# ps-auxw/CLI-P

Hardware: AMD Instinct MI355X
Metric: images/sec ViT-B/32 encode (higher is better)
Workload: dtype bf16

## Files before the change

cli-p_amd/_lib.py:

```python
import ctypes as C
import os

HERE = os.path.dirname(os.path.abspath(__file__))
DEV_LIB = os.environ.get("CLIPMI_DEV_LIB", "") not in ("", "0")
LIB_PATH = os.path.join(HERE, "libclipmi_dev.so" if DEV_LIB else "libclipmi.so")

ABI_VERSION = 8
F32, BF16, U8 = 0, 1, 2

SYMBOLS = [
    "clipmi_encode_image_workspace_bytes", "clipmi_encode_image",
    "clipmi_encode_text_workspace_bytes", "clipmi_encode_text",
    "clipmi_topk_ip_workspace_bytes", "clipmi_topk_ip",
    "clipmi_topk_ip_coarse_workspace_bytes", "clipmi_topk_ip_coarse", "clipmi_dbg_topk_coarse_scan_ms",
    "clipmi_rows_stats", "clipmi_rows_absmax", "clipmi_rows_order_workspace_bytes", "clipmi_rows_order_by_absmax", "clipmi_rows_to_bf16", "clipmi_i8_copy_bytes", "clipmi_i8_meta_bytes", "clipmi_quantize_rows_i8", "clipmi_topk_ip_coarse_i8", "clipmi_dbg_topk_coarse_i8_scan_ms",
    "clipmi_topk_ip_wide_workspace_bytes", "clipmi_topk_ip_wide_i8", "clipmi_dbg_topk_wide_i8_scan_ms",
    "clipmi_dbg_quantize_rows_fp8", "clipmi_dbg_gemm_fp8",
    "clipmi_merge_topk_workspace_bytes", "clipmi_merge_topk", "clipmi_merge_topk_packed",
    "clipmi_l2_normalize_rows", "clipmi_resize_crop_rgb8", "clipmi_jpeg_workspace_bytes", "clipmi_jpeg_decode_rgb8", "clipmi_jpeg_progressive_workspace_bytes", "clipmi_jpeg_decode_progressive_rgb8", "clipmi_png_workspace_bytes", "clipmi_png_decode_rgb8", "clipmi_last_error", "clipmi_abi_version",
    "clipmi_dbg_gemm_bf16", "clipmi_dbg_layernorm", "clipmi_dbg_attention", "clipmi_dbg_topk_scan_ms",
    "clipmi_dbg_encode_image_probe_ms", "clipmi_dbg_encode_image_probe3_ms",
    "clipmi_dbg_split_stats", "clipmi_dbg_gemm_ln", "clipmi_dbg_gemm_resid_ln", "clipmi_dbg_gemm_resid_ln_leaf", "clipmi_dbg_gemm_ln_leaf", "clipmi_dbg_quantize_rows_fp8mx", "clipmi_dbg_gemm_fp8_bsa",
]


class Tower(C.Structure):
    _fields_ = [(n, C.c_int32) for n in (
        "abi_version", "kind", "width", "layers", "heads", "mlp", "embed", "tokens",
        "patch", "res", "patch_k", "vocab")] + [(n, C.c_uint64) for n in (
        "blob_bytes",
        "off_patch_w", "off_cls", "off_pos", "off_ln_pre_w", "off_ln_pre_b",
        "off_tok_emb",
        "off_layers", "layer_stride",
        "lo_ln1_w", "lo_ln1_b", "lo_qkv_w", "lo_qkv_b", "lo_out_w", "lo_out_b",
        "lo_ln2_w", "lo_ln2_b", "lo_fc_w", "lo_fc_b", "lo_proj_w", "lo_proj_b",
        "off_ln_post_w", "off_ln_post_b", "off_out_proj")] + [
        ("weight_format", C.c_int32), ("ln_fold", C.c_int32)] + [(n, C.c_uint64) for n in (
        "lo_qkv_s", "lo_out_s", "lo_fc_s", "lo_proj_s", "lo_qkv_colsum", "lo_qkv_cb", "lo_fc_colsum", "lo_fc_cb")]


class ClipmiError(RuntimeError):
    pass

# ... 93 lines not shown
    L.clipmi_png_workspace_bytes.argtypes = [i32, i64]
    L.clipmi_png_decode_rgb8.restype = i32
    L.clipmi_png_decode_rgb8.argtypes = [vp, vp, i32, i64, i64, vp, vp, vp, i64, vp]
    L.clipmi_dbg_gemm_bf16.restype = i32
    L.clipmi_dbg_gemm_bf16.argtypes = [vp, vp, vp, vp, i32, i32, i32, i32, vp]
    L.clipmi_dbg_split_stats.restype = i32
    L.clipmi_dbg_split_stats.argtypes = [vp, i32, vp, vp, i32, i32, vp]
    L.clipmi_dbg_gemm_ln.restype = i32
    L.clipmi_dbg_gemm_ln.argtypes = [vp, vp, vp, vp, vp, vp, i32, i32, i32, i32, vp]
    L.clipmi_dbg_quantize_rows_fp8mx.restype = i32
    L.clipmi_dbg_quantize_rows_fp8mx.argtypes = [vp, vp, vp, i32, i32, vp]
    L.clipmi_dbg_gemm_fp8_bsa.restype = i32
    L.clipmi_dbg_gemm_fp8_bsa.argtypes = [vp, vp, vp, vp, vp, vp, i32, i32, i32, i32, vp]
    L.clipmi_dbg_gemm_resid_ln_leaf.restype = i32
    L.clipmi_dbg_gemm_resid_ln_leaf.argtypes = [vp, vp, vp, vp, vp, i32, i32, i32, vp]
    L.clipmi_dbg_gemm_ln_leaf.restype = i32
    L.clipmi_dbg_gemm_ln_leaf.argtypes = [vp, vp, vp, vp, vp, vp, i32, i32, i32, i32, vp]
    L.clipmi_dbg_gemm_resid_ln.restype = i32
    L.clipmi_dbg_gemm_resid_ln.argtypes = [vp, vp, vp, vp, vp, vp, i32, i32, i32, i32, vp]
    L.clipmi_dbg_layernorm.restype = i32
    L.clipmi_dbg_layernorm.argtypes = [vp, vp, vp, vp, i32, i32, i32, vp]
    L.clipmi_dbg_attention.restype = i32
    L.clipmi_dbg_attention.argtypes = [vp, vp, i32, i32, i32, i32, vp]
    L.clipmi_dbg_topk_scan_ms.restype = i32
    L.clipmi_dbg_topk_scan_ms.argtypes = [vp, i64, i32, vp, i32, i32, vp, vp, vp, sz, vp, i32, C.POINTER(C.c_float)]
    L.clipmi_dbg_encode_image_probe_ms.restype = i32
    L.clipmi_dbg_encode_image_probe_ms.argtypes = [TP, vp, vp, i32, i32, vp, vp, sz, vp, i32, i32,
                                                   C.POINTER(C.c_float), C.POINTER(C.c_int)]
    L.clipmi_dbg_encode_image_probe3_ms.restype = i32
    L.clipmi_dbg_encode_image_probe3_ms.argtypes = [TP, vp, vp, i32, i32, vp, vp, sz, vp, i32, i32,
                                                    C.POINTER(C.c_float), C.POINTER(C.c_int), C.POINTER(C.c_int),
                                                    C.POINTER(C.c_int)]
    if L.clipmi_abi_version() != ABI_VERSION:
        raise ClipmiError(f"libclipmi.so ABI {L.clipmi_abi_version()} != binding {ABI_VERSION}: rebuild")
    _lib = L
    return L


def check(rc, what):
    if rc != 0:
        msg = lib().clipmi_last_error().decode("utf-8", "replace")
        raise ClipmiError(f"{what} failed (code {rc}): {msg}")


def last_error():
    return lib().clipmi_last_error().decode("utf-8", "replace")
# ... 31 lines not shown
```

cli-p_amd/csrc/encode.hip:

```cpp
#include "vit_kernels.hpp"

namespace clipmi {
namespace {

struct Ws {
    unsigned short* patches;
    float* x;
    unsigned short* h;
    unsigned short* big;
    unsigned short* pooled;
    int* rowidx;
    unsigned char* a8;
    float* a_scale;
    unsigned char* a_bs;
    unsigned char* x8;
    unsigned char* x8_bs;
    void* x3;
    float* ln_part;
    float* ln_leaf;
    void* x3c;
    float* partc;
    float* leafc;
    float* xc;
};

size_t carve(const clipmi_tower* t, int B, void* base, size_t cap, Ws* out) {
    Arena ar(base ? base : reinterpret_cast<void*>(256), cap);
    const size_t rows = (size_t)B * t->tokens;
    const int W = t->width;
    Ws w{};
    if (t->kind == 0) w.patches = ar.take<unsigned short>((size_t)B * (t->tokens - 1) * t->patch_k);
    w.x = ar.take<float>(rows * W);
    w.h = ar.take<unsigned short>(rows * W);
    w.big = ar.take<unsigned short>(rows * 4 * W);
    w.pooled = ar.take<unsigned short>((size_t)B * W);
    w.rowidx = ar.take<int>((size_t)B);
    if (t->weight_format == 1) {
        w.a8 = ar.take<unsigned char>(rows * 4 * W);
        w.a_scale = ar.take<float>(rows);
        w.a_bs = ar.take<unsigned char>((rows + 255) / 256 * 256 * (size_t)(4 * W / 32));
    }
    if (t->ln_fold && t->weight_format == 1) {
        w.x8 = ar.take<unsigned char>(rows * W);
        w.x8_bs = ar.take<unsigned char>((rows + 255) / 256 * 256 * (size_t)(W / 32));
        w.ln_part = ar.take<float>(rows * 2 * (W / 256));
    } else if (t->ln_fold) {
        w.x3 = ar.take<unsigned char>(rows * resid_row_bytes(W));
        w.ln_part = ar.take<float>(rows * 2 * (W / 256));
        if (rows <= (size_t)SKINNY_MAX_M) w.ln_leaf = ar.take<float>(rows * 2 * (W / 4));
    }
    if (t->kind == 0 && t->weight_format == 0) {
        if (t->ln_fold) {
            w.x3c = ar.take<unsigned char>((size_t)B * resid_row_bytes(W));
            w.partc = ar.take<float>((size_t)B * 2 * (W / 256));
            if (B <= SKINNY_MAX_M) w.leafc = ar.take<float>((size_t)B * 2 * (W / 4));
        } else {
            w.xc = ar.take<float>((size_t)B * W);
        }
    }
    if (out) *out = w;
    return ar.off + 256;
}

int check_tower(const clipmi_tower* t, int kind, const char* who) {
    if (!t) return set_err(CLIPMI_EINVAL, "%s: NULL tower", who);
    if (t->abi_version != CLIPMI_ABI_VERSION)
        return set_err(CLIPMI_EINVAL, "%s: tower ABI %d != %d", who, t->abi_version, CLIPMI_ABI_VERSION);
    if (t->kind != kind) return set_err(CLIPMI_EINVAL, "%s: tower kind %d", who, t->kind);
    if (t->width % 128 != 0 || t->heads * 64 != t->width || t->mlp != 4 * t->width || t->embed % 128 != 0 ||
        t->width > 1024 || t->layers < 1)
        return set_err(CLIPMI_EUNSUPPORTED,
                       "%s: width=%d heads=%d mlp=%d embed=%d (need width %% 128 == 0 <= 1024, head dim 64, embed %% 128 == 0)",
                       who, t->width, t->heads, t->mlp, t->embed);
    if (t->weight_format != 0 && t->weight_format != 1)
        return set_err(CLIPMI_EINVAL, "%s: weight_format %d", who, t->weight_format);
    if (t->weight_format == 1 && t->width % 256 != 0)
        return set_err(CLIPMI_EUNSUPPORTED, "%s: fp8 weights need width %% 256 == 0 (width %d)", who, t->width);
    if (t->ln_fold != 0 && (t->ln_fold != 1 || t->width % 256 != 0))
        return set_err(CLIPMI_EINVAL, "%s: ln_fold %d needs width %% 256 == 0 (width %d)", who, t->ln_fold, t->width);
#ifndef CLIPMI_DEV
    if (t->ln_fold != 0 && t->weight_format != 0)
        return set_err(CLIPMI_EUNSUPPORTED, "%s: folded LayerNorms on FP8 weights exist in the development library only", who);
#endif
    if (t->tokens > 80 && kind == 1)
        return set_err(CLIPMI_EUNSUPPORTED, "%s: %d tokens (causal attention covers <= 80)", who, t->tokens);
    return 0;
}

template <typename T>
const T* at(const void* blob, uint64_t off) {
    return reinterpret_cast<const T*>(static_cast<const char*>(blob) + off);
}

bool encode_tail() {
    static const int mode = (int)dev_knob("CLIPMI_ENCODE_TAIL", 1);
    return mode != 0;
}

int launch_gather_rows(const void* src, void* dst, int B, int L, size_t row_bytes, hipStream_t st) {
    if (row_bytes % 16 != 0) return set_err(CLIPMI_EINVAL, "gather_rows: %zu bytes per row", row_bytes);
    const int row16 = (int)(row_bytes / 16);
    hipLaunchKernelGGL(gather_rows_kernel, dim3((unsigned)(((long long)B * row16 + 255) / 256)), dim3(256), 0, st,
                       static_cast<const uint4*>(src), static_cast<uint4*>(dst), B, L, row16);
    CLIPMI_CHECK_LAUNCH("gather_rows_kernel");
    return 0;
}

int run_layers(const clipmi_tower* t, const void* blob, const Ws& w, int B, int causal, hipStream_t st, GemmProbe* probe,
               bool* pruned = nullptr) {
    const int W = t->width, L = t->tokens, M = B * L;
    const bool fp8 = t->weight_format == 1;
    const bool tail = pruned && !causal && !fp8 && (t->ln_fold ? w.x3c != nullptr : w.xc != nullptr) && encode_tail();
    if (pruned) *pruned = tail;
    auto linear = [&](const unsigned short* A, int K, uint64_t w_off, uint64_t b_off, void* out, int N, int epi) -> int {
        GemmArgs g{};
        g.bias = at<float>(blob, b_off); g.out = out; g.M = M; g.N = N; g.K = K;
        g.A = A; g.W = at<unsigned short>(blob, w_off);
        return launch_gemm_algo(g, epi, 0, st, probe);
    };
#ifdef CLIPMI_DEV
    if (t->ln_fold && fp8) {
        auto lnfold8 = [&](uint64_t w_off, uint64_t s_off, uint64_t cb_off, uint64_t cs_off, void* out, unsigned char* out_bs, int N,
                           int epi) -> int {
            GemmArgs g{};
            g.A = reinterpret_cast<const unsigned short*>(w.x8); g.a_bscale = w.x8_bs;
            g.W = at<unsigned short>(blob, w_off); g.w_scale = at<float>(blob, s_off);
            g.bias = at<float>(blob, cb_off); g.colsum = at<float>(blob, cs_off); g.ln_part_in = w.ln_part;
// ... 32 lines not shown
    if (t->ln_fold) {
        auto lb_of = [&](int l) { return t->off_layers + (uint64_t)l * t->layer_stride; };
        const bool leaf_mode = w.ln_leaf != nullptr && gemm_resid_writes_leaves(M, W, W) && gemm_resid_writes_leaves(M, W, 4 * W);
        bool leaves = false;
        auto ln_linear = [&](uint64_t w_off, uint64_t cb_off, uint64_t cs_off, int N, int epi) -> int {
            GemmArgs g{};
            g.A = static_cast<const unsigned short*>(w.x3); g.lda_bytes = (unsigned)resid_row_bytes(W);
            g.W = at<unsigned short>(blob, w_off); g.bias = at<float>(blob, cb_off);
            g.colsum = at<float>(blob, cs_off); g.ln_part_in = w.ln_part;
            if (leaves) g.ln_leaf_in = w.ln_leaf;
            g.out = w.big; g.M = M; g.N = N; g.K = W;
            return launch_gemm_algo(g, epi, 0, st, probe);
        };
        auto resid_linear = [&](const unsigned short* A, int K, uint64_t w_off, uint64_t b_off) -> int {
            GemmArgs g{};
            g.A = A; g.W = at<unsigned short>(blob, w_off); g.bias = at<float>(blob, b_off);
            g.M = M; g.N = W; g.K = K;
            g.x3 = w.x3; g.ln_part = w.ln_part; g.tmp_f32 = w.x;
            if (leaf_mode) { g.ln_leaf = w.ln_leaf; leaves = true; }
            return launch_gemm_algo(g, EPI_BIAS_RESID_LN_F32, 0, st, probe);
        };
        for (int l = 0; l < t->layers; ++l) {
            const uint64_t lb = lb_of(l);
            if (int rc = ln_linear(lb + t->lo_qkv_w, lb + t->lo_qkv_cb, lb + t->lo_qkv_colsum, 3 * W, EPI_LN_BIAS_BF16)) return rc;
            if (tail && l == t->layers - 1) {
                const bool tleaf = w.leafc != nullptr && gemm_resid_writes_leaves(B, W, W) && gemm_resid_writes_leaves(B, W, 4 * W);
                if (int rc = launch_attention(w.big, w.h, B, L, t->heads, causal, 1, st)) return rc;
                if (int rc = launch_gather_rows(w.x3, w.x3c, B, L, resid_row_bytes(W), st)) return rc;
                auto tail_resid = [&](const unsigned short* A, unsigned lda_bytes, int K, uint64_t w_off, uint64_t b_off) -> int {
                    GemmArgs g{};
                    g.A = A; g.lda_bytes = lda_bytes; g.W = at<unsigned short>(blob, w_off); g.bias = at<float>(blob, b_off);
                    g.M = B; g.N = W; g.K = K;
                    g.x3 = w.x3c; g.ln_part = w.partc; g.tmp_f32 = w.x;
                    if (tleaf) g.ln_leaf = w.leafc;
                    return launch_gemm_algo(g, EPI_BIAS_RESID_LN_F32, 0, st, nullptr);
                };
                if (int rc = tail_resid(w.h, (unsigned)((size_t)L * W * 2), W, lb + t->lo_out_w, lb + t->lo_out_b)) return rc;
                GemmArgs g{};
                g.A = static_cast<const unsigned short*>(w.x3c); g.lda_bytes = (unsigned)resid_row_bytes(W);
                g.W = at<unsigned short>(blob, lb + t->lo_fc_w); g.bias = at<float>(blob, lb + t->lo_fc_cb);
                g.colsum = at<float>(blob, lb + t->lo_fc_colsum); g.ln_part_in = w.partc;
                if (tleaf) g.ln_leaf_in = w.leafc;
                g.out = w.big; g.M = B; g.N = 4 * W; g.K = W;
                if (int rc = launch_gemm_algo(g, EPI_LN_BIAS_QGELU_BF16, 0, st, nullptr)) return rc;
                return tail_resid(w.big, 0u, 4 * W, lb + t->lo_proj_w, lb + t->lo_proj_b);
            }
            hipEvent_t* aev = nullptr;
            if (probe && probe->mode == 2 && probe->n < GemmProbe::MAX) {
                const int pi = probe->begin(GemmProbe::EPI_ATTENTION, 2, st, 0);
                aev = &probe->ev[2 * pi];
            }
// ... 256 lines not shown
```

cli-p_amd/csrc/vit_kernels.hip:

```cpp
#include "vit_kernels.hpp"
#include <hip/hip_ext.h>
#include <cstdlib>

namespace clipmi {

int launch_layernorm(const LnArgs& a, hipStream_t st) {
    if (a.M < 1) return 0;
    if (a.W % 4 != 0 || a.W > 1024) return set_err(CLIPMI_EINVAL, "layernorm: W=%d (need W %% 4 == 0, W <= 1024)", a.W);
    if (a.out_x3 && (a.W % 256 != 0 || !a.out_part)) return set_err(CLIPMI_EINVAL, "layernorm: split output needs W %% 256 == 0");
    hipLaunchKernelGGL(layernorm_kernel, dim3((a.M + 3) / 4), dim3(256), 0, st, a);
    CLIPMI_CHECK_LAUNCH("layernorm_kernel");
    return 0;
}

int launch_split_stats(const float* x_or_add, bool add, void* x3, float* part, int M, int W, hipStream_t st) {
    if (M < 1) return 0;
    if (!x_or_add || !x3 || !part || W % 256 != 0 || W < 256 || W > 1024)
        return set_err(CLIPMI_EINVAL, "split_stats: W=%d (need W %% 256 == 0, 256 <= W <= 1024)", W);
    if (add) hipLaunchKernelGGL(split_stats_kernel<true>, dim3((M + 3) / 4), dim3(256), 0, st, x_or_add, x3, part, M, W);
    else hipLaunchKernelGGL(split_stats_kernel<false>, dim3((M + 3) / 4), dim3(256), 0, st, x_or_add, x3, part, M, W);
    CLIPMI_CHECK_LAUNCH("split_stats_kernel");
    return 0;
}

template <int NT, bool CAUSAL, bool TR>
static int launch_attn_t(const unsigned short* qkv, unsigned short* out, int B, int L, int heads, hipStream_t st) {
    constexpr int KS = (NT + 1) / 2;
    const size_t lds = 4 * KS * 32 * 128;
    const long long items = (long long)B * heads;
    hipLaunchKernelGGL((attention_kernel<NT, CAUSAL, TR>), dim3((unsigned)((items + 3) / 4)), dim3(256), lds, st, qkv, out,
                       B, L, heads);
    CLIPMI_CHECK_LAUNCH("attention_kernel");
    return 0;
}

int launch_attention(const unsigned short* qkv, unsigned short* out, int B, int L, int heads, int causal, int tr,
                     hipStream_t st, unsigned char* out8, unsigned char* out_bs, bool* fused, hipEvent_t* probe_ev) {
    if (fused) *fused = false;
    if (B < 1) return 0;
    if (L < 1) return set_err(CLIPMI_EINVAL, "attention: L=%d", L);
    if (L > 80) {
        if (causal) return set_err(CLIPMI_EUNSUPPORTED, "attention: causal mask with L=%d > 80", L);
        const int qblocks = (L + 31) / 32;
        const int g4 = (qblocks + 3) / 4;
        const long long groups = (long long)B * heads * g4;
        hipLaunchKernelGGL((attention_flash_kernel<4, 2>), dim3((unsigned)groups), dim3(256), 2 * 16384, st, qkv, out, B, L, heads, g4);
        CLIPMI_CHECK_LAUNCH("attention_flash_kernel");
        return 0;
    }
    const int nt = (L + 15) / 16;
    static const int use52 = (int)dev_knob("CLIPMI_ATTN52", 2);
    if (L >= 49 && L <= 52 && !causal && tr == 1 && use52 == 2) {
        const long long items = (long long)B * heads;
        const long long resident = (long long)NUM_CU * 5;
        if (out8 && out_bs && fused) {
            hipLaunchKernelGGL(attention52x4_kernel<true>, dim3((unsigned)(items < resident ? items : resident)), dim3(256),
                               64 * 128 + 52 * 128, st, qkv, out, B, L, heads, out8, out_bs);
            *fused = true;
        } else if (probe_ev) {
            hipExtLaunchKernelGGL(attention52x4_kernel<false>, dim3((unsigned)(items < resident ? items : resident)), dim3(256),
                                  64 * 128 + 52 * 128, st, probe_ev[0], probe_ev[1], 0, qkv, out, B, L, heads, (unsigned char*)nullptr,
                                  (unsigned char*)nullptr);
        } else {
            hipLaunchKernelGGL(attention52x4_kernel<false>, dim3((unsigned)(items < resident ? items : resident)), dim3(256),
                               64 * 128 + 52 * 128, st, qkv, out, B, L, heads, (unsigned char*)nullptr, (unsigned char*)nullptr);
        }
        CLIPMI_CHECK_LAUNCH("attention52x4_kernel");
        return 0;
    }
    if (L >= 49 && L <= 52 && !causal && tr && use52) {
        const long long items = (long long)B * heads;
        const size_t lds = 4 * 52 * 128;
        hipLaunchKernelGGL(attention52_kernel, dim3((unsigned)((items + 3) / 4)), dim3(256), lds, st, qkv, out, B, L, heads);
        CLIPMI_CHECK_LAUNCH("attention52_kernel");
        return 0;
    }
#define ATT(NT_)                                                                                         \
    if (nt <= NT_) {                                                                                     \
        if (causal) return tr ? launch_attn_t<NT_, true, true>(qkv, out, B, L, heads, st)                \
                              : launch_attn_t<NT_, true, false>(qkv, out, B, L, heads, st);              \
        return tr ? launch_attn_t<NT_, false, true>(qkv, out, B, L, heads, st)                           \
                  : launch_attn_t<NT_, false, false>(qkv, out, B, L, heads, st);                         \
    }
    ATT(1) ATT(2) ATT(4) ATT(5)
#undef ATT
    return set_err(CLIPMI_EUNSUPPORTED, "attention: L=%d", L);
}

// ... 33 lines not shown
    hipLaunchKernelGGL(patchify_kernel, dim3((unsigned)((total + 255) / 256)), dim3(256), 0, st, a);
    CLIPMI_CHECK_LAUNCH("patchify_kernel");
    return 0;
}

}

using namespace clipmi;

extern "C" int clipmi_dbg_layernorm(const float* x_dev, const float* w_dev, const float* b_dev, void* out_dev, int M,
                                    int W, int out_bf16, void* stream) {
    if (!x_dev || !w_dev || !b_dev || !out_dev) return set_err(CLIPMI_EINVAL, "dbg_layernorm: NULL pointer");
    LnArgs a{x_dev, w_dev, b_dev, out_dev, nullptr, 1, M, W, out_bf16};
    return launch_layernorm(a, as_stream(stream));
}

extern "C" int clipmi_dbg_attention(const void* qkv_dev, void* out_dev, int B, int L, int heads, int causal,
                                    void* stream) {
    if (!qkv_dev || !out_dev) return set_err(CLIPMI_EINVAL, "dbg_attention: NULL pointer");
    return launch_attention(static_cast<const unsigned short*>(qkv_dev), static_cast<unsigned short*>(out_dev), B, L,
                            heads, causal & 1, (causal & 2) ? 0 : ((causal & 4) ? 2 : 1), as_stream(stream));
}

extern "C" int clipmi_dbg_quantize_rows_fp8(const void* in_bf16_dev, void* out_fp8_dev, float* scale_dev, int M, int K,
                                            void* stream) {
    return launch_quantize_rows_fp8(static_cast<const unsigned short*>(in_bf16_dev), static_cast<unsigned char*>(out_fp8_dev),
                                    scale_dev, M, K, as_stream(stream));
}

extern "C" int clipmi_dbg_quantize_rows_fp8mx(const void* in_bf16_dev, void* out_fp8_dev, void* bscale_dev, int M, int K, void* stream) {
    return launch_quantize_rows_fp8mx(static_cast<const unsigned short*>(in_bf16_dev), static_cast<unsigned char*>(out_fp8_dev),
                                      static_cast<unsigned char*>(bscale_dev), M, K, as_stream(stream));
}

extern "C" int clipmi_dbg_split_stats(const float* x_dev, int add, void* x3_dev, float* part_dev, int M, int W, void* stream) {
    return launch_split_stats(x_dev, add != 0, x3_dev, part_dev, M, W, as_stream(stream));
}
```

cli-p_amd/csrc/vit_kernels.hpp:

```cpp
#pragma once
#include "gemm.hpp"

namespace clipmi {

struct PatchArgs {
    const void* pix;
    unsigned short* out;
    int dtype, B, R, P, grid, np, patch_k;
};

static __global__ void __launch_bounds__(256) patchify_kernel(PatchArgs a) {
    const long long total = (long long)a.B * a.np * (a.patch_k / 8);
    const long long i = (long long)blockIdx.x * 256 + threadIdx.x;
    if (i >= total) return;
    const int kc = a.patch_k / 8;
    const int k8 = (int)(i % kc);
    const long long bp = i / kc;
    const int p = (int)(bp % a.np);
    const int b = (int)(bp / a.np);
    const int PP = a.P * a.P;
    const float mean[3] = {0.48145466f, 0.4578275f, 0.40821073f};
    const float stdv[3] = {0.26862954f, 0.26130258f, 0.27577711f};
    float v[8];
    if ((a.P & 7) == 0 && (a.R & 7) == 0) {
// ... 76 lines not shown
            const unsigned b0 = (word >> (16 * (k & 1))) & 0xffu, b1 = (word >> (16 * (k & 1) + 8)) & 0xffu;
            w4[k] = (unsigned)lut[b0] | ((unsigned)lut[b1] << 16);
        }
        unsigned short* dst = a.out + ((size_t)b * a.np + gy * a.grid + gx) * a.patch_k + c * a.P * a.P + y * a.P + px;
        *reinterpret_cast<uint4*>(dst) = make_uint4(w4[0], w4[1], w4[2], w4[3]);
    }
}

static __global__ void __launch_bounds__(256) cls_rows_kernel(float* x, const float* cls, const float* pos, int B, int L, int W) {
    const long long i = (long long)blockIdx.x * 256 + threadIdx.x;
    if (i >= (long long)B * W) return;
    const int b = (int)(i / W), c = (int)(i - (long long)b * W);
    x[(size_t)b * L * W + c] = cls[c] + pos[c];
}

static __global__ void __launch_bounds__(256) gather_rows_kernel(const uint4* __restrict__ src, uint4* __restrict__ dst, int B,
                                                                 int row_step, int row16) {
    const long long i = (long long)blockIdx.x * 256 + threadIdx.x;
    if (i >= (long long)B * row16) return;
    const int b = (int)(i / row16), c = (int)(i - (long long)b * row16);
    dst[(size_t)b * row16 + c] = src[(size_t)b * row_step * row16 + c];
}

static __global__ void __launch_bounds__(256) text_embed_kernel(float* x, const int* ids, const float* tok, const float* pos,
                                                         int Q, int L, int W, int vocab) {
    const long long i = (long long)blockIdx.x * 256 + threadIdx.x;
    const int wc = W / 4;
    if (i >= (long long)Q * L * wc) return;
    const int c4 = (int)(i % wc);
    const long long row = i / wc;
    const int t = (int)(row % L);
    int id = ids[row];
    id = id < 0 ? 0 : (id >= vocab ? vocab - 1 : id);
    const f32x4 e = *reinterpret_cast<const f32x4*>(tok + (size_t)id * W + c4 * 4);
    const f32x4 p = *reinterpret_cast<const f32x4*>(pos + (size_t)t * W + c4 * 4);
    *reinterpret_cast<f32x4*>(x + (size_t)row * W + c4 * 4) = e + p;
}

static __global__ void eot_rows_kernel(const int* ids, int* rowidx, int Q, int L) {
    const int q = blockIdx.x * blockDim.x + threadIdx.x;
    if (q >= Q) return;
    int best = ids[(size_t)q * L], bi = 0;
    for (int t = 1; t < L; ++t) {
        const int v = ids[(size_t)q * L + t];
        if (v > best) { best = v; bi = t; }
    }
// ... 518 lines not shown
                                       pack_bf16x2(hi.z, hi.w));
            const bf16x8 pf = __builtin_bit_cast(bf16x8, u);
#pragma unroll
            for (int dt = 0; dt < 4; ++dt) {
                const s16x4 t0 = __builtin_amdgcn_ds_read_tr16_b64_v4i16(
                    (__attribute__((address_space(3))) s16x4*)(vcol + krow[2 * ks] * 128 + dt * 32));
                const s16x4 t1 = __builtin_amdgcn_ds_read_tr16_b64_v4i16(
                    (__attribute__((address_space(3))) s16x4*)(vcol + krow[2 * ks + 1] * 128 + dt * 32));
                typedef short s16x8 __attribute__((ext_vector_type(8)));
                const s16x8 t = {t0.x, t0.y, t0.z, t0.w, t1.x, t1.y, t1.z, t1.w};
                o[dt] = __builtin_amdgcn_mfma_f32_16x16x32_bf16(__builtin_bit_cast(bf16x8, t), pf, o[dt], 0, 0, 0);
            }
        }
        const int qi = qt * 16 + fr;
        if (qi < L) {
            unsigned short* dst = out + ((size_t)b * L + qi) * W + h * 64 + 4 * fg;
#pragma unroll
            for (int dt = 0; dt < 4; ++dt)
                *reinterpret_cast<uint2*>(dst + dt * 16) = make_uint2(pack_bf16x2(o[dt].x, o[dt].y), pack_bf16x2(o[dt].z, o[dt].w));
        }
    }
}

template <bool OUT8>
static __global__ void __launch_bounds__(256, 5) attention52x4_kernel(const unsigned short* __restrict__ qkv,
                                                                      unsigned short* __restrict__ out, int B, int L,
                                                                      int heads, unsigned char* __restrict__ out8, unsigned char* __restrict__ out_bs) {
    extern __shared__ __attribute__((aligned(16))) char smem[];
    constexpr int NT = 4, ROWS = 52;
    const int lane = threadIdx.x & 63;
    const int wave = __builtin_amdgcn_readfirstlane(threadIdx.x >> 6);
    const int fr = lane & 15, fg = lane >> 4;
    const int W = heads * 64;
    const size_t rs = (size_t)3 * W;
    char* kt_ = smem;
    char* vt = smem + 64 * 128;
    const int srow = lane >> 3, sch = lane & 7;
    const int items = B * heads;

    bf16x8 q0n, q1n;
    uint4 kdn0, kdn1, vdn0, vdn1;
#define ATT52_FETCH(IT)                                                                                  \
    do {                                                                                                 \
        const int b_ = (IT) / heads, h_ = (IT) - b_ * heads;                                             \
        const unsigned short* base_ = qkv + (size_t)b_ * L * 3 * W + h_ * 64;                            \
        int qrow_ = wave * 16 + fr;                                                                      \
        qrow_ = qrow_ < L ? qrow_ : L - 1;                                                               \
        const unsigned short* qp_ = base_ + (size_t)qrow_ * rs + fg * 8;                                 \
        q0n = *reinterpret_cast<const bf16x8*>(qp_);                                                     \
        q1n = *reinterpret_cast<const bf16x8*>(qp_ + 32);                                                \
        int r0_ = (wave * 2) * 8 + srow, r1_ = (wave * 2 + 1) * 8 + srow;    \
        r0_ = r0_ < L ? r0_ : L - 1;                                         \
        r1_ = r1_ < L ? r1_ : L - 1;                                                                     \
        kdn0 = *reinterpret_cast<const uint4*>(base_ + (size_t)r0_ * rs + W + sch * 8);                  \
        vdn0 = *reinterpret_cast<const uint4*>(base_ + (size_t)r0_ * rs + 2 * W + sch * 8);              \
        kdn1 = *reinterpret_cast<const uint4*>(base_ + (size_t)r1_ * rs + W + sch * 8);                  \
        vdn1 = *reinterpret_cast<const uint4*>(base_ + (size_t)r1_ * rs + 2 * W + sch * 8);              \
    } while (0)
    int item = blockIdx.x;
    if (item >= items) return;
    ATT52_FETCH(item);
    for (;;) {
        const int b = item / heads, h = item - b * heads;
        const bf16x8 q0 = q0n, q1 = q1n;
        {
            const int row0 = (wave * 2) * 8 + srow, row1 = row0 + 8;
            *reinterpret_cast<uint4*>(kt_ + row0 * 128 + ((sch ^ (row0 & 7)) << 4)) = kdn0;
            *reinterpret_cast<uint4*>(kt_ + row1 * 128 + ((sch ^ (row1 & 7)) << 4)) = kdn1;
            if (row0 < ROWS) *reinterpret_cast<uint4*>(vt + row0 * 128 + sch * 16) = vdn0;
            if (row1 < ROWS) *reinterpret_cast<uint4*>(vt + row1 * 128 + sch * 16) = vdn1;
        }
        const int nxt = item + gridDim.x;
        const bool has_next = nxt < items;
        if (has_next) ATT52_FETCH(nxt);
        __syncthreads();

    bf16x8 kf[NT][2];
#pragma unroll
    for (int t = 0; t < NT; ++t) {
        const int row = t * 16 + fr;
        kf[t][0] = *reinterpret_cast<const bf16x8*>(kt_ + row * 128 + (((0 + fg) ^ (row & 7)) << 4));
        kf[t][1] = *reinterpret_cast<const bf16x8*>(kt_ + row * 128 + (((4 + fg) ^ (row & 7)) << 4));
    }
    const int k00 = 4 * fg + (fr >> 2);
    const int krow[4] = {k00, k00 + 16, k00 + 32, (k00 + 48 < ROWS ? k00 + 48 : ROWS - 1)};
    const char* vcol = vt + (4 * (fr & 3)) * 2;

    f32x4 s[NT];
#pragma unroll
    for (int kt = 0; kt < NT; ++kt) {
        f32x4 a = {0.f, 0.f, 0.f, 0.f};
        a = __builtin_amdgcn_mfma_f32_16x16x32_bf16(kf[kt][0], q0, a, 0, 0, 0);
        a = __builtin_amdgcn_mfma_f32_16x16x32_bf16(kf[kt][1], q1, a, 0, 0, 0);
        s[kt] = a;
    }
    float mx = -INFINITY;
#pragma unroll
    for (int kt = 0; kt < NT; ++kt)
#pragma unroll
// ... 60 lines not shown
            const uint4 v = odd ? make_uint4(theirs[j].x, theirs[j].y, mine[j].x, mine[j].y)
                                : make_uint4(mine[j].x, mine[j].y, theirs[j].x, theirs[j].y);
            const unsigned w_[4] = {v.x, v.y, v.z, v.w};
            float f[8];
            float mxa = 0.f;
#pragma unroll
            for (int i = 0; i < 4; ++i) {
                f[2 * i] = __uint_as_float(w_[i] << 16);
                f[2 * i + 1] = __uint_as_float(w_[i] & 0xffff0000u);
                mxa = fmaxf(mxa, fmaxf(fabsf(f[2 * i]), fabsf(f[2 * i + 1])));
            }
            mxa = fmaxf(mxa, __shfl_xor(mxa, 16));
            mxa = fmaxf(mxa, __shfl_xor(mxa, 32));
            const unsigned sb_ = fp8mx_scale_byte(mxa);
            const float inv_ = fp8mx_inv(sb_);
#pragma unroll
            for (int i = 0; i < 8; ++i) f[i] *= inv_;
            if (qi < L) {
                const size_t row_ = (size_t)b * L + qi;
                *reinterpret_cast<uint2*>(out8 + row_ * W + h * 64 + 4 * (fg & ~1) + dt * 16) = fp8_pack8(f);
                if (fg == 0) out_bs[row_ * (W >> 5) + h * 2 + j] = (unsigned char)sb_;
            }
        }
    } else if (qi < L) {
        unsigned short* dst = out + ((size_t)b * L + qi) * W + h * 64 + 4 * (fg & ~1);
#pragma unroll
        for (int j = 0; j < 2; ++j) {
            const int dt = 2 * j + (odd ? 1 : 0);
            const uint4 v = odd ? make_uint4(theirs[j].x, theirs[j].y, mine[j].x, mine[j].y)
                                : make_uint4(mine[j].x, mine[j].y, theirs[j].x, theirs[j].y);
            *reinterpret_cast<uint4*>(dst + dt * 16) = v;
        }
    }
        if (!has_next) break;
        item = nxt;
        __syncthreads();
    }
#undef ATT52_FETCH
}

template <int WPB, int QT>
__global__ void __launch_bounds__(WPB * 64, QT == 2 ? 4 : 2) attention_flash_kernel(const unsigned short* __restrict__ qkv,
                                                                    unsigned short* __restrict__ out, int B, int L,
                                                                    int heads, int qgroups) {
    extern __shared__ __attribute__((aligned(16))) char smem[];
    constexpr int NT = 4;
    const int tid = threadIdx.x;
    const int lane = tid & 63;
    const int wave = __builtin_amdgcn_readfirstlane(tid >> 6);
    const int fr = lane & 15, fg = lane >> 4;
    const int W = heads * 64;
    const int qgi = blockIdx.x % qgroups;
    const int bh = blockIdx.x / qgroups;
    const int b = bh / heads, h = bh - b * heads;
    const unsigned short* base = qkv + (size_t)b * L * 3 * W + h * 64;
// ... 137 lines not shown
    for (int j = 0; j + 1 < nb; ++j) block(std::false_type{}, j);
    if ((nb << 6) > L) block(std::true_type{}, nb - 1);
    else block(std::false_type{}, nb - 1);

    if (!wave_active) return;
#pragma unroll
    for (int qt = 0; qt < QT; ++qt) {
        const int qi = q0 + qt * 16 + fr;
        if (qi >= L) continue;
        const float inv = 1.0f / l_run[qt];
        unsigned short* dst = out + ((size_t)b * L + qi) * W + h * 64 + 4 * fg;
#pragma unroll
        for (int dt = 0; dt < 4; ++dt) {
            const f32x4 v = o[dt][qt] * inv;
            *reinterpret_cast<uint2*>(dst + dt * 16) = make_uint2(pack_bf16x2(v.x, v.y), pack_bf16x2(v.z, v.w));
        }
    }
}

int launch_layernorm(const LnArgs& a, hipStream_t st);
int launch_attention(const unsigned short* qkv, unsigned short* out, int B, int L, int heads, int causal, int tr,
                     hipStream_t st, unsigned char* out8 = nullptr, unsigned char* out_bs = nullptr, bool* fused = nullptr,
                     hipEvent_t* probe_ev = nullptr);
int launch_patchify(const PatchArgs& a, hipStream_t st);
int launch_quantize_rows_fp8(const unsigned short* in, unsigned char* out, float* scale, int M, int K, hipStream_t st);
int launch_quantize_rows_fp8mx(const unsigned short* in, unsigned char* out, unsigned char* bscale, int M, int K, hipStream_t st);
int launch_rows_mx_stats(const float* x, unsigned char* x8, unsigned char* bs, float* part, int M, int W, hipStream_t st);

}
```

include/clipmi.h:

```cpp
#ifndef CLIPMI_H
#define CLIPMI_H

#include <stddef.h>
#include <stdint.h>

#ifdef __cplusplus
extern "C" {
#endif

#define CLIPMI_ABI_VERSION 8

enum {
    CLIPMI_OK = 0,
    CLIPMI_EINVAL = 1,
    CLIPMI_EWORKSPACE = 2,
    CLIPMI_EHIP = 3,
    CLIPMI_EUNSUPPORTED = 4
};

enum {
    CLIPMI_F32 = 0,
    CLIPMI_BF16 = 1,
    CLIPMI_U8 = 2
};
// ... 149 lines not shown

typedef struct clipmi_png_image {
    int64_t stream_off;
    int64_t raw_off;
    int64_t out_off;
    int32_t stream_bytes;
    int32_t width, height;
    int32_t channels;
    int32_t reserved[2];
} clipmi_png_image;
int64_t clipmi_png_workspace_bytes(int n, int64_t total_raw_bytes);
int clipmi_png_decode_rgb8(const void* streams_dev, const void* images_dev, int n, int64_t total_raw_bytes, int64_t max_raw_bytes,
                           void* out_dev, int32_t* status_dev, void* ws_dev, int64_t ws_bytes, void* stream);

const char* clipmi_last_error(void);
int clipmi_abi_version(void);

int clipmi_dbg_gemm_bf16(const void* a_dev, const void* w_dev, const float* bias_dev,
                         void* out_dev, int M, int N, int K, int epi, void* stream);
int clipmi_dbg_layernorm(const float* x_dev, const float* w_dev, const float* b_dev,
                         void* out_dev, int M, int W, int out_bf16, void* stream);
int clipmi_dbg_attention(const void* qkv_dev, void* out_dev, int B, int L, int heads,
                         int causal, void* stream);

int clipmi_dbg_topk_scan_ms(const void* db_dev, int64_t N, int E, const float* q_dev, int Q, int K,
                            float* out_score_dev, int64_t* out_id_dev, void* ws_dev, size_t ws_bytes,
                            void* stream, int reps, float* scan_ms);

int clipmi_dbg_topk_coarse_scan_ms(const void* db_dev, const void* db_bf16_dev, int64_t N, int E, float rmax,
                                   const float* q_dev, int Q, int K, float* out_score_dev, int64_t* out_id_dev,
                                   void* ws_dev, size_t ws_bytes, void* stream, int reps, float* scan_ms,
                                   long long* survivors );

int clipmi_dbg_topk_coarse_i8_scan_ms(const void* db_dev, const void* db_i8_dev, const float* meta_dev, float amax,
                                      int64_t N, int E, float rmax, const float* q_dev, int Q, int K,
                                      float* out_score_dev, int64_t* out_id_dev, void* ws_dev, size_t ws_bytes,
                                      void* stream, int reps, float* scan_ms, long long* survivors);

int clipmi_dbg_topk_wide_i8_scan_ms(const void* db_dev, const void* db_i8_dev, const float* meta_dev, float amax,
                                    int64_t N, int E, float rmax, const float* q_dev, int Q, int K,
                                    float* out_score_dev, int64_t* out_id_dev, void* ws_dev, size_t ws_bytes,
                                    void* stream, int reps, float* scan_ms, long long* survivors, int* scan_launches,
                                    int* fallback_armed);

int clipmi_dbg_quantize_rows_fp8(const void* in_bf16_dev, void* out_fp8_dev, float* scale_dev, int M, int K, void* stream);
int clipmi_dbg_gemm_fp8(const void* a8_dev, const void* w8_dev, const float* a_scale_dev, const float* w_scale_dev,
// ... 29 lines not shown
```

Before: 111,400.

## Compute only the class-token query in the last layer's attention

In the final encoder layer only the class row is needed downstream. The Q projection is therefore computed just for the gathered class rows, together with their LN statistics, while K/V are projected for all tokens. A class-only variant of the 52-token attention kernel then computes and writes only row 0 per image. This removes about a third of the last layer's QKV GEMM work and most of its attention work, at the cost of an extra GEMM launch and a gather kernel that also copies the statistics.

```diff
diff --git a/cli-p_amd/_lib.py b/cli-p_amd/_lib.py
--- a/cli-p_amd/_lib.py
+++ b/cli-p_amd/_lib.py
@@ -18,7 +18,7 @@
     "clipmi_dbg_quantize_rows_fp8", "clipmi_dbg_gemm_fp8",
     "clipmi_merge_topk_workspace_bytes", "clipmi_merge_topk", "clipmi_merge_topk_packed",
     "clipmi_l2_normalize_rows", "clipmi_resize_crop_rgb8", "clipmi_jpeg_workspace_bytes", "clipmi_jpeg_decode_rgb8", "clipmi_jpeg_progressive_workspace_bytes", "clipmi_jpeg_decode_progressive_rgb8", "clipmi_png_workspace_bytes", "clipmi_png_decode_rgb8", "clipmi_last_error", "clipmi_abi_version",
-    "clipmi_dbg_gemm_bf16", "clipmi_dbg_layernorm", "clipmi_dbg_attention", "clipmi_dbg_topk_scan_ms",
+    "clipmi_dbg_gemm_bf16", "clipmi_dbg_layernorm", "clipmi_dbg_attention", "clipmi_dbg_attention_cls", "clipmi_dbg_topk_scan_ms",
     "clipmi_dbg_encode_image_probe_ms", "clipmi_dbg_encode_image_probe3_ms",
     "clipmi_dbg_split_stats", "clipmi_dbg_gemm_ln", "clipmi_dbg_gemm_resid_ln", "clipmi_dbg_gemm_resid_ln_leaf", "clipmi_dbg_gemm_ln_leaf", "clipmi_dbg_quantize_rows_fp8mx", "clipmi_dbg_gemm_fp8_bsa",
 ]
@@ -158,6 +158,8 @@
     L.clipmi_dbg_layernorm.argtypes = [vp, vp, vp, vp, i32, i32, i32, vp]
     L.clipmi_dbg_attention.restype = i32
     L.clipmi_dbg_attention.argtypes = [vp, vp, i32, i32, i32, i32, vp]
+    L.clipmi_dbg_attention_cls.restype = i32
+    L.clipmi_dbg_attention_cls.argtypes = [vp, vp, vp, i32, i32, i32, vp]
     L.clipmi_dbg_topk_scan_ms.restype = i32
     L.clipmi_dbg_topk_scan_ms.argtypes = [vp, i64, i32, vp, i32, i32, vp, vp, vp, sz, vp, i32, C.POINTER(C.c_float)]
     L.clipmi_dbg_encode_image_probe_ms.restype = i32
diff --git a/cli-p_amd/csrc/encode.hip b/cli-p_amd/csrc/encode.hip
--- a/cli-p_amd/csrc/encode.hip
+++ b/cli-p_amd/csrc/encode.hip
@@ -21,6 +21,7 @@
     void* x3c;
     float* partc;
     float* leafc;
+    unsigned short* qc;
     float* xc;
 };
 
@@ -54,6 +55,7 @@
             w.x3c = ar.take<unsigned char>((size_t)B * resid_row_bytes(W));
             w.partc = ar.take<float>((size_t)B * 2 * (W / 256));
             if (B <= SKINNY_MAX_M) w.leafc = ar.take<float>((size_t)B * 2 * (W / 4));
+            w.qc = ar.take<unsigned short>((size_t)B * W);
         } else {
             w.xc = ar.take<float>((size_t)B * W);
         }
@@ -97,12 +99,27 @@
     return mode != 0;
 }
 
+bool encode_clsq() {
+    static const int mode = (int)dev_knob("CLIPMI_ENCODE_CLSQ", 1);
+    return mode != 0;
+}
+
 int launch_gather_rows(const void* src, void* dst, int B, int L, size_t row_bytes, hipStream_t st) {
     if (row_bytes % 16 != 0) return set_err(CLIPMI_EINVAL, "gather_rows: %zu bytes per row", row_bytes);
     const int row16 = (int)(row_bytes / 16);
     hipLaunchKernelGGL(gather_rows_kernel, dim3((unsigned)(((long long)B * row16 + 255) / 256)), dim3(256), 0, st,
                        static_cast<const uint4*>(src), static_cast<uint4*>(dst), B, L, row16);
     CLIPMI_CHECK_LAUNCH("gather_rows_kernel");
+    return 0;
+}
+
+int launch_gather_cls(const void* x3, void* x3c, const float* stat, float* statc, int B, int L, int W, int stat_pairs, hipStream_t st) {
+    const int row16 = (int)(resid_row_bytes(W) / 16);
+    if (resid_row_bytes(W) % 16 != 0 || !x3 || !x3c || !stat || !statc) return set_err(CLIPMI_EINVAL, "gather_cls: W=%d", W);
+    hipLaunchKernelGGL(gather_cls_kernel, dim3((unsigned)(((long long)B * (row16 + stat_pairs) + 255) / 256)), dim3(256), 0, st,
+                       static_cast<const uint4*>(x3), static_cast<uint4*>(x3c), reinterpret_cast<const uint2*>(stat),
+                       reinterpret_cast<uint2*>(statc), B, L, row16, stat_pairs);
+    CLIPMI_CHECK_LAUNCH("gather_cls_kernel");
     return 0;
 }
 
@@ -181,11 +198,36 @@
         };
         for (int l = 0; l < t->layers; ++l) {
             const uint64_t lb = lb_of(l);
-            if (int rc = ln_linear(lb + t->lo_qkv_w, lb + t->lo_qkv_cb, lb + t->lo_qkv_colsum, 3 * W, EPI_LN_BIAS_BF16)) return rc;
-            if (tail && l == t->layers - 1) {
+            const bool last = tail && l == t->layers - 1;
+            const bool clsq = last && w.qc != nullptr && attention_has_cls_form(L, causal) && encode_clsq();
+            if (!clsq)
+                if (int rc = ln_linear(lb + t->lo_qkv_w, lb + t->lo_qkv_cb, lb + t->lo_qkv_colsum, 3 * W, EPI_LN_BIAS_BF16)) return rc;
+            if (last) {
                 const bool tleaf = w.leafc != nullptr && gemm_resid_writes_leaves(B, W, W) && gemm_resid_writes_leaves(B, W, 4 * W);
-                if (int rc = launch_attention(w.big, w.h, B, L, t->heads, causal, 1, st)) return rc;
-                if (int rc = launch_gather_rows(w.x3, w.x3c, B, L, resid_row_bytes(W), st)) return rc;
+                if (clsq) {
+                    const bool cleaf = leaves && w.leafc != nullptr;
+                    if (leaves && !cleaf) return set_err(CLIPMI_EINVAL, "encode_image: statistics leaves without a class-row buffer");
+                    if (int rc = launch_gather_cls(w.x3, w.x3c, cleaf ? w.ln_leaf : w.ln_part, cleaf ? w.leafc : w.partc, B, L, W,
+                                                   cleaf ? W / 4 : W / 256, st)) return rc;
+                    GemmArgs q{};
+                    q.A = static_cast<const unsigned short*>(w.x3c); q.lda_bytes = (unsigned)resid_row_bytes(W);
+                    q.W = at<unsigned short>(blob, lb + t->lo_qkv_w); q.bias = at<float>(blob, lb + t->lo_qkv_cb);
+                    q.colsum = at<float>(blob, lb + t->lo_qkv_colsum);
+                    if (cleaf) q.ln_leaf_in = w.leafc; else q.ln_part_in = w.partc;
+                    q.out = w.qc; q.M = B; q.N = W; q.K = W;
+                    if (int rc = launch_gemm_algo(q, EPI_LN_BIAS_BF16, 0, st, nullptr)) return rc;
+                    GemmArgs kv{};
+                    kv.A = static_cast<const unsigned short*>(w.x3); kv.lda_bytes = (unsigned)resid_row_bytes(W);
+                    kv.W = at<unsigned short>(blob, lb + t->lo_qkv_w) + (size_t)W * W; kv.bias = at<float>(blob, lb + t->lo_qkv_cb) + W;
+                    kv.colsum = at<float>(blob, lb + t->lo_qkv_colsum) + W; kv.ln_part_in = w.ln_part;
+                    if (leaves) kv.ln_leaf_in = w.ln_leaf;
+                    kv.out = w.big; kv.M = M; kv.N = 2 * W; kv.K = W;
+                    if (int rc = launch_gemm_algo(kv, EPI_LN_BIAS_BF16, 0, st, nullptr)) return rc;
+                    if (int rc = launch_attention_cls(w.qc, w.big, w.h, B, L, t->heads, st)) return rc;
+                } else {
+                    if (int rc = launch_attention(w.big, w.h, B, L, t->heads, causal, 1, st)) return rc;
+                    if (int rc = launch_gather_rows(w.x3, w.x3c, B, L, resid_row_bytes(W), st)) return rc;
+                }
                 auto tail_resid = [&](const unsigned short* A, unsigned lda_bytes, int K, uint64_t w_off, uint64_t b_off) -> int {
                     GemmArgs g{};
                     g.A = A; g.lda_bytes = lda_bytes; g.W = at<unsigned short>(blob, w_off); g.bias = at<float>(blob, b_off);
diff --git a/cli-p_amd/csrc/vit_kernels.hip b/cli-p_amd/csrc/vit_kernels.hip
--- a/cli-p_amd/csrc/vit_kernels.hip
+++ b/cli-p_amd/csrc/vit_kernels.hip
@@ -34,6 +34,25 @@
     return 0;
 }
 
+static int attn52_mode() {
+    static const int use52 = (int)dev_knob("CLIPMI_ATTN52", 2);
+    return use52;
+}
+
+bool attention_has_cls_form(int L, int causal) { return L >= 49 && L <= 52 && !causal && attn52_mode() == 2; }
+
+int launch_attention_cls(const unsigned short* qcls, const unsigned short* kv, unsigned short* out, int B, int L, int heads,
+                         hipStream_t st) {
+    if (B < 1) return 0;
+    if (!attention_has_cls_form(L, 0)) return set_err(CLIPMI_EUNSUPPORTED, "attention_cls: L=%d (49 <= L <= 52)", L);
+    const long long items = (long long)B * heads;
+    const long long resident = (long long)NUM_CU * 5;
+    hipLaunchKernelGGL((attention52x4_kernel<false, true>), dim3((unsigned)(items < resident ? items : resident)), dim3(256),
+                       64 * 128 + 52 * 128, st, kv, out, B, L, heads, (unsigned char*)nullptr, (unsigned char*)nullptr, qcls);
+    CLIPMI_CHECK_LAUNCH("attention52x4_kernel<cls>");
+    return 0;
+}
+
 int launch_attention(const unsigned short* qkv, unsigned short* out, int B, int L, int heads, int causal, int tr,
                      hipStream_t st, unsigned char* out8, unsigned char* out_bs, bool* fused, hipEvent_t* probe_ev) {
     if (fused) *fused = false;
@@ -49,21 +68,22 @@
         return 0;
     }
     const int nt = (L + 15) / 16;
-    static const int use52 = (int)dev_knob("CLIPMI_ATTN52", 2);
+    const int use52 = attn52_mode();
     if (L >= 49 && L <= 52 && !causal && tr == 1 && use52 == 2) {
         const long long items = (long long)B * heads;
         const long long resident = (long long)NUM_CU * 5;
         if (out8 && out_bs && fused) {
             hipLaunchKernelGGL(attention52x4_kernel<true>, dim3((unsigned)(items < resident ? items : resident)), dim3(256),
-                               64 * 128 + 52 * 128, st, qkv, out, B, L, heads, out8, out_bs);
+                               64 * 128 + 52 * 128, st, qkv, out, B, L, heads, out8, out_bs, (const unsigned short*)nullptr);
             *fused = true;
         } else if (probe_ev) {
             hipExtLaunchKernelGGL(attention52x4_kernel<false>, dim3((unsigned)(items < resident ? items : resident)), dim3(256),
                                   64 * 128 + 52 * 128, st, probe_ev[0], probe_ev[1], 0, qkv, out, B, L, heads, (unsigned char*)nullptr,
-                                  (unsigned char*)nullptr);
+                                  (unsigned char*)nullptr, (const unsigned short*)nullptr);
         } else {
             hipLaunchKernelGGL(attention52x4_kernel<false>, dim3((unsigned)(items < resident ? items : resident)), dim3(256),
-                               64 * 128 + 52 * 128, st, qkv, out, B, L, heads, (unsigned char*)nullptr, (unsigned char*)nullptr);
+                               64 * 128 + 52 * 128, st, qkv, out, B, L, heads, (unsigned char*)nullptr, (unsigned char*)nullptr,
+                               (const unsigned short*)nullptr);
         }
         CLIPMI_CHECK_LAUNCH("attention52x4_kernel");
         return 0;
@@ -143,6 +163,14 @@
                             heads, causal & 1, (causal & 2) ? 0 : ((causal & 4) ? 2 : 1), as_stream(stream));
 }
 
+extern "C" int clipmi_dbg_attention_cls(const void* q_dev, const void* kv_dev, void* out_dev, int B, int L, int heads,
+                                        void* stream) {
+    if (!q_dev || !kv_dev || !out_dev) return set_err(CLIPMI_EINVAL, "dbg_attention_cls: NULL pointer");
+    if (heads < 1) return set_err(CLIPMI_EINVAL, "dbg_attention_cls: heads=%d", heads);
+    return launch_attention_cls(static_cast<const unsigned short*>(q_dev), static_cast<const unsigned short*>(kv_dev),
+                                static_cast<unsigned short*>(out_dev), B, L, heads, as_stream(stream));
+}
+
 extern "C" int clipmi_dbg_quantize_rows_fp8(const void* in_bf16_dev, void* out_fp8_dev, float* scale_dev, int M, int K,
                                             void* stream) {
     return launch_quantize_rows_fp8(static_cast<const unsigned short*>(in_bf16_dev), static_cast<unsigned char*>(out_fp8_dev),
diff --git a/cli-p_amd/csrc/vit_kernels.hpp b/cli-p_amd/csrc/vit_kernels.hpp
--- a/cli-p_amd/csrc/vit_kernels.hpp
+++ b/cli-p_amd/csrc/vit_kernels.hpp
@@ -122,6 +122,17 @@
     dst[(size_t)b * row16 + c] = src[(size_t)b * row_step * row16 + c];
 }
 
+static __global__ void __launch_bounds__(256) gather_cls_kernel(const uint4* __restrict__ src, uint4* __restrict__ dst,
+                                                                const uint2* __restrict__ ssrc, uint2* __restrict__ sdst, int B,
+                                                                int row_step, int row16, int stat2) {
+    const long long i = (long long)blockIdx.x * 256 + threadIdx.x;
+    const int per = row16 + stat2;
+    if (i >= (long long)B * per) return;
+    const int b = (int)(i / per), c = (int)(i - (long long)b * per);
+    if (c < row16) dst[(size_t)b * row16 + c] = src[(size_t)b * row_step * row16 + c];
+    else sdst[(size_t)b * stat2 + (c - row16)] = ssrc[(size_t)b * row_step * stat2 + (c - row16)];
+}
+
 static __global__ void __launch_bounds__(256) text_embed_kernel(float* x, const int* ids, const float* tok, const float* pos,
                                                          int Q, int L, int W, int vocab) {
     const long long i = (long long)blockIdx.x * 256 + threadIdx.x;
@@ -686,17 +697,20 @@
     }
 }
 
-template <bool OUT8>
+template <bool OUT8, bool CLS = false>
 static __global__ void __launch_bounds__(256, 5) attention52x4_kernel(const unsigned short* __restrict__ qkv,
                                                                       unsigned short* __restrict__ out, int B, int L,
-                                                                      int heads, unsigned char* __restrict__ out8, unsigned char* __restrict__ out_bs) {
+                                                                      int heads, unsigned char* __restrict__ out8, unsigned char* __restrict__ out_bs,
+                                                                      const unsigned short* __restrict__ qcls) {
+    static_assert(!(OUT8 && CLS), "the class-only form writes bf16 rows");
     extern __shared__ __attribute__((aligned(16))) char smem[];
     constexpr int NT = 4, ROWS = 52;
     const int lane = threadIdx.x & 63;
     const int wave = __builtin_amdgcn_readfirstlane(threadIdx.x >> 6);
     const int fr = lane & 15, fg = lane >> 4;
     const int W = heads * 64;
-    const size_t rs = (size_t)3 * W;
+    const size_t rs = (size_t)(CLS ? 2 : 3) * W;
+    const int kcol = CLS ? 0 : W, vcol0 = CLS ? W : 2 * W;
     char* kt_ = smem;
     char* vt = smem + 64 * 128;
     const int srow = lane >> 3, sch = lane & 7;
@@ -707,19 +721,28 @@
 #define ATT52_FETCH(IT)                                                                                  \
     do {                                                                                                 \
         const int b_ = (IT) / heads, h_ = (IT) - b_ * heads;                                             \
-        const unsigned short* base_ = qkv + (size_t)b_ * L * 3 * W + h_ * 64;                            \
-        int qrow_ = wave * 16 + fr;                                                                      \
-        qrow_ = qrow_ < L ? qrow_ : L - 1;                                                               \
-        const unsigned short* qp_ = base_ + (size_t)qrow_ * rs + fg * 8;                                 \
-        q0n = *reinterpret_cast<const bf16x8*>(qp_);                                                     \
-        q1n = *reinterpret_cast<const bf16x8*>(qp_ + 32);                                                \
+        const unsigned short* base_ = qkv + (size_t)b_ * L * rs + h_ * 64;                               \
+        if (CLS) {                           \
+            q0n = q1n = __builtin_bit_cast(bf16x8, make_uint4(0u, 0u, 0u, 0u));                          \
+            if (wave == 0 && fr == 0) {                                                                  \
+                const unsigned short* qp_ = qcls + (size_t)b_ * W + h_ * 64 + fg * 8;                    \
+                q0n = *reinterpret_cast<const bf16x8*>(qp_);                                             \
+                q1n = *reinterpret_cast<const bf16x8*>(qp_ + 32);                                        \
+            }                                                                                            \
+        } else {                                                                                         \
+            int qrow_ = wave * 16 + fr;                                                                  \
+            qrow_ = qrow_ < L ? qrow_ : L - 1;                                                           \
+            const unsigned short* qp_ = base_ + (size_t)qrow_ * rs + fg * 8;                             \
+            q0n = *reinterpret_cast<const bf16x8*>(qp_);                                                 \
+            q1n = *reinterpret_cast<const bf16x8*>(qp_ + 32);                                            \
+        }                                                                                                \
         int r0_ = (wave * 2) * 8 + srow, r1_ = (wave * 2 + 1) * 8 + srow;    \
         r0_ = r0_ < L ? r0_ : L - 1;                                         \
         r1_ = r1_ < L ? r1_ : L - 1;                                                                     \
-        kdn0 = *reinterpret_cast<const uint4*>(base_ + (size_t)r0_ * rs + W + sch * 8);                  \
-        vdn0 = *reinterpret_cast<const uint4*>(base_ + (size_t)r0_ * rs + 2 * W + sch * 8);              \
-        kdn1 = *reinterpret_cast<const uint4*>(base_ + (size_t)r1_ * rs + W + sch * 8);                  \
-        vdn1 = *reinterpret_cast<const uint4*>(base_ + (size_t)r1_ * rs + 2 * W + sch * 8);              \
+        kdn0 = *reinterpret_cast<const uint4*>(base_ + (size_t)r0_ * rs + kcol + sch * 8);               \
+        vdn0 = *reinterpret_cast<const uint4*>(base_ + (size_t)r0_ * rs + vcol0 + sch * 8);              \
+        kdn1 = *reinterpret_cast<const uint4*>(base_ + (size_t)r1_ * rs + kcol + sch * 8);               \
+        vdn1 = *reinterpret_cast<const uint4*>(base_ + (size_t)r1_ * rs + vcol0 + sch * 8);              \
     } while (0)
     int item = blockIdx.x;
     if (item >= items) return;
@@ -739,6 +762,7 @@
         if (has_next) ATT52_FETCH(nxt);
         __syncthreads();
 
+    if (!CLS || wave == 0) {
     bf16x8 kf[NT][2];
 #pragma unroll
     for (int t = 0; t < NT; ++t) {
@@ -845,7 +869,7 @@
                 if (fg == 0) out_bs[row_ * (W >> 5) + h * 2 + j] = (unsigned char)sb_;
             }
         }
-    } else if (qi < L) {
+    } else if (CLS ? qi == 0 : qi < L) {
         unsigned short* dst = out + ((size_t)b * L + qi) * W + h * 64 + 4 * (fg & ~1);
 #pragma unroll
         for (int j = 0; j < 2; ++j) {
@@ -854,6 +878,7 @@
                                 : make_uint4(mine[j].x, mine[j].y, theirs[j].x, theirs[j].y);
             *reinterpret_cast<uint4*>(dst + dt * 16) = v;
         }
+    }
     }
         if (!has_next) break;
         item = nxt;
@@ -1037,6 +1062,9 @@
 int launch_attention(const unsigned short* qkv, unsigned short* out, int B, int L, int heads, int causal, int tr,
                      hipStream_t st, unsigned char* out8 = nullptr, unsigned char* out_bs = nullptr, bool* fused = nullptr,
                      hipEvent_t* probe_ev = nullptr);
+bool attention_has_cls_form(int L, int causal);
+int launch_attention_cls(const unsigned short* qcls, const unsigned short* kv, unsigned short* out, int B, int L, int heads,
+                         hipStream_t st);
 int launch_patchify(const PatchArgs& a, hipStream_t st);
 int launch_quantize_rows_fp8(const unsigned short* in, unsigned char* out, float* scale, int M, int K, hipStream_t st);
 int launch_quantize_rows_fp8mx(const unsigned short* in, unsigned char* out, unsigned char* bscale, int M, int K, hipStream_t st);
diff --git a/include/clipmi.h b/include/clipmi.h
--- a/include/clipmi.h
+++ b/include/clipmi.h
@@ -195,6 +195,8 @@
                          void* out_dev, int M, int W, int out_bf16, void* stream);
 int clipmi_dbg_attention(const void* qkv_dev, void* out_dev, int B, int L, int heads,
                          int causal, void* stream);
+int clipmi_dbg_attention_cls(const void* q_dev, const void* kv_dev, void* out_dev, int B, int L,
+                             int heads, void* stream);
 
 int clipmi_dbg_topk_scan_ms(const void* db_dev, int64_t N, int E, const float* q_dev, int Q, int K,
                             float* out_score_dev, int64_t* out_id_dev, void* ws_dev, size_t ws_bytes,
```

Result: no change. 111,600, median of 6 (+0.2%).
